# tsurumeso/vocal-remover

Measured on NVIDIA H100. Metric: seconds-of-audio/sec separated (n_fft=2048, hop=1024), higher is better.
Workload: dtype bf16x3 (split-bf16 operands hi+lo, 3 wgmma passes, fp32 accumulate); fft/lstm fp32

## Files before the change

vocal-remover_b200/build.py:

```python
import os
import subprocess
import sys
from concurrent.futures import ThreadPoolExecutor

HERE = os.path.dirname(os.path.abspath(__file__))
CSRC = os.path.join(HERE, 'csrc')
OBJ = os.path.join(HERE, 'build')
LIB = os.path.join(HERE, 'libvr_b200.so')
SOURCES = ['api.cu', 'engine.cu', 'conv_simt.cu', 'conv_tc.cu', 'conv_tc_rows.cu', 'conv_tc_halo.cu', 'elementwise.cu', 'lstm.cu', 'fft.cu', 'resample.cu']
NVCC = os.environ.get('NVCC', '/usr/local/cuda/bin/nvcc')
FLAGS = ['-gencode', 'arch=compute_90a,code=sm_90a', '-O3', '-lineinfo', '-std=c++17',
         '-Xcompiler', '-fPIC', '-Xcompiler', '-fvisibility=hidden', '--expt-relaxed-constexpr']


def _newest_header():
    hs = [os.path.join(CSRC, f) for f in os.listdir(CSRC) if f.endswith(('.h', '.cuh'))]
    hs.append(os.path.join(HERE, '..', 'include', 'vr_b200.h'))
    return max(os.path.getmtime(h) for h in hs)


def build(verbose=False, force=False):
    global OBJ, LIB
    extra = os.environ.get('VR_BUILD_FLAGS', '').split()
    if os.environ.get('VR_BUILD_TAG'):
        OBJ = os.path.join(HERE, 'build_' + os.environ['VR_BUILD_TAG'])
        LIB = os.path.join(HERE, 'libvr_b200_%s.so' % os.environ['VR_BUILD_TAG'])
    os.makedirs(OBJ, exist_ok=True)
    hdr = _newest_header()
    jobs = []
    for src in SOURCES:
        s = os.path.join(CSRC, src)
        o = os.path.join(OBJ, src.replace('.cu', '.o'))
        if force or not os.path.exists(o) or os.path.getmtime(o) < max(os.path.getmtime(s), hdr):
            jobs.append((s, o))

    def cc(job):
        s, o = job
        cmd = [NVCC] + FLAGS + extra + ['-c', s, '-o', o]
        if verbose:
            cmd += ['-Xptxas', '-v']
        r = subprocess.run(cmd, capture_output=True, text=True)
        if r.returncode != 0:
            raise RuntimeError('nvcc failed for %s:\n%s\n%s' % (s, r.stdout, r.stderr))
        return r.stderr

    with ThreadPoolExecutor(max_workers=min(8, max(1, len(jobs)))) as ex:
        logs = list(ex.map(cc, jobs))
    if verbose:
        for lg in logs:
            print(lg)
    objs = [os.path.join(OBJ, s.replace('.cu', '.o')) for s in SOURCES]
    if jobs or not os.path.exists(LIB):
        cmd = [NVCC, '-shared', '-o', LIB] + objs + ['-gencode', 'arch=compute_90a,code=sm_90a']
        r = subprocess.run(cmd, capture_output=True, text=True)
        if r.returncode != 0:
            raise RuntimeError('link failed:\n%s\n%s' % (r.stdout, r.stderr))
    return LIB


if __name__ == '__main__':
    print(build(verbose='-v' in sys.argv, force='-f' in sys.argv))
```

vocal-remover_b200/csrc/api.cu:

```cuda
#include <stdio.h>
#include <string.h>

#include <string>

#include "../../include/vr_b200.h"
#include "engine.h"
#include "kernels.h"
#include "tc_plan.h"

struct vr_ctx {
  vr::Engine* eng;
  std::string err;
};

static std::string g_create_err;

static int fail(vr_ctx* c, const std::string& m) {
  if (c) c->err = m;
  return -1;
}
static int done(vr_ctx* c, bool ok) {
  if (ok) return 0;
  c->err = c->eng->err;
  return -1;
}
#define CHECK_CTX(c) \
  if (!(c) || !(c)->eng) return -2;

extern "C" {

int vr_create(const vr_config* cfg, vr_ctx** out) {
  if (!cfg || !out) return -2;
  *out = nullptr;
  int ndev = 0;
  if (cudaGetDeviceCount(&ndev) != cudaSuccess || ndev == 0) {
    g_create_err = "no CUDA device visible: libvr_b200 has no CPU path";
    return -1;
  }
  if (cfg->device < 0 || cfg->device >= ndev) {
    g_create_err = "invalid device ordinal";
    return -1;
  }
  int nf = cfg->n_fft;
  if (nf < 64 || nf > 4096 || (nf & (nf - 1))) {
    g_create_err = "n_fft must be a power of two in [64, 4096]";
    return -1;
  }
  if (cfg->hop_length <= 0 || cfg->hop_length > nf) {
    g_create_err = "hop_length must be in (0, n_fft]";
    return -1;
  }
  if (cfg->max_batch <= 0 || cfg->cropsize <= 0) {
    g_create_err = "max_batch and cropsize must be positive";
    return -1;
  }
  vr::Config c;
  c.device = cfg->device; c.n_fft = cfg->n_fft; c.hop = cfg->hop_length; c.nout = cfg->nout;
  c.nout_lstm = cfg->nout_lstm; c.cropsize = cfg->cropsize; c.max_batch = cfg->max_batch;
  c.conv_mode = cfg->conv_mode;
  vr_ctx* ctx = new vr_ctx();
  ctx->eng = new vr::Engine(c);
  if (!ctx->eng->err.empty()) {
    g_create_err = ctx->eng->err;
    delete ctx->eng;
    delete ctx;
    return -1;
  }
  *out = ctx;
  return 0;
}

void vr_destroy(vr_ctx* ctx) {
  if (!ctx) return;
  delete ctx->eng;
  delete ctx;
}

const char* vr_last_error(const vr_ctx* ctx) { return ctx ? ctx->err.c_str() : g_create_err.c_str(); }

int vr_load_tensor(vr_ctx* ctx, const char* name, int32_t dtype, int32_t ndim, const int64_t* shape,
                   const void* host_data) {
  CHECK_CTX(ctx);
  if (!name || (!host_data) || ndim < 0 || ndim > 8) return fail(ctx, "vr_load_tensor: bad arguments");
  return done(ctx, ctx->eng->load_tensor(name, dtype, ndim, shape, host_data));
}

int vr_finalize_weights(vr_ctx* ctx) {
  CHECK_CTX(ctx);
  return done(ctx, ctx->eng->finalize());
}

int vr_stft(vr_ctx* ctx, const float* wave, int64_t L, void* spec, int64_t T, float* absmax, void* stream) {
  CHECK_CTX(ctx);
  return done(ctx, ctx->eng->stft(wave, L, (float2*)spec, T, absmax, (cudaStream_t)stream));
}

int vr_istft(vr_ctx* ctx, const void* spec, int64_t T, float* wave, void* stream) {
  CHECK_CTX(ctx);
  return done(ctx, ctx->eng->istft((const float2*)spec, nullptr, T, wave, nullptr, (cudaStream_t)stream));
}

int vr_predict_mask(vr_ctx* ctx, const float* mag, int32_t N, float* mask, void* stream) {
  CHECK_CTX(ctx);
  return done(ctx, ctx->eng->predict_mask(mag, N, mask, ctx->eng->cfg().offset, (cudaStream_t)stream));
}

int vr_forward(vr_ctx* ctx, const float* mag, int32_t N, float* mask, void* stream) {
  CHECK_CTX(ctx);
  return done(ctx, ctx->eng->predict_mask(mag, N, mask, 0, (cudaStream_t)stream));
}

int vr_normaliser(vr_ctx* ctx, const void* spec, int64_t T, int32_t norm_mode, float* out, void* stream) {
  CHECK_CTX(ctx);
  return done(ctx, ctx->eng->normaliser((const float2*)spec, T, norm_mode, out, (cudaStream_t)stream));
}

int vr_separate_windows(vr_ctx* ctx, const void* spec, int64_t T, const float* norm, int32_t pad_l,
                        int32_t first_window, int32_t n_windows, float* mask, int64_t mask_T, int64_t frame_shift,
                        int32_t accumulate, void* stream) {
  CHECK_CTX(ctx);
  return done(ctx, ctx->eng->separate_windows((const float2*)spec, T, norm, pad_l, first_window, n_windows, mask,
                                              mask_T, frame_shift, accumulate, (cudaStream_t)stream));
}

int vr_separate(vr_ctx* ctx, const void* spec, int64_t T, int32_t tta, float* mask, void* stream) {
  CHECK_CTX(ctx);
  return done(ctx, ctx->eng->separate((const float2*)spec, T, tta, mask, (cudaStream_t)stream));
}

int vr_apply_mask(vr_ctx* ctx, const void* spec, const float* mask, int64_t T, void* y_spec, void* v_spec,
                  void* stream) {
  CHECK_CTX(ctx);
  return done(ctx, ctx->eng->apply_mask((const float2*)spec, mask, T, (float2*)y_spec, (float2*)v_spec,
                                        (cudaStream_t)stream));
}

int vr_mask_frame_min(vr_ctx* ctx, const float* mask, int64_t T, float* frame_min, void* stream) {
  CHECK_CTX(ctx);
  return done(ctx, ctx->eng->mask_frame_min(mask, T, frame_min, (cudaStream_t)stream));
}

int vr_mask_apply_weight(vr_ctx* ctx, float* mask, int64_t T, const float* weight, void* stream) {
  CHECK_CTX(ctx);
  return done(ctx, ctx->eng->mask_apply_weight(mask, T, weight, (cudaStream_t)stream));
}

int vr_apply_mask_istft(vr_ctx* ctx, const void* spec, const float* mask, int64_t T, float* wave_inst,
                        float* wave_voc, void* stream) {
  CHECK_CTX(ctx);
  if (!mask) return fail(ctx, "vr_apply_mask_istft: mask is NULL");
  return done(ctx, ctx->eng->istft((const float2*)spec, mask, T, wave_inst, wave_voc, (cudaStream_t)stream));
}

int vr_stft_range(vr_ctx* ctx, const float* wave, int64_t L, void* spec, int64_t T, int64_t t0, int64_t t1,
                  void* stream) {
  CHECK_CTX(ctx);
  return done(ctx, ctx->eng->stft_range(wave, L, (float2*)spec, T, t0, t1, (cudaStream_t)stream));
}

int vr_normaliser_range(vr_ctx* ctx, const void* spec, int64_t T, int64_t t0, int64_t t1, float* out, void* stream) {
  CHECK_CTX(ctx);
  return done(ctx, ctx->eng->normaliser_range((const float2*)spec, T, t0, t1, out, (cudaStream_t)stream));
}

int vr_apply_mask_istft_range(vr_ctx* ctx, const void* spec, const float* mask, int64_t T, int64_t k0, int64_t k1,
                              float* wave_inst, float* wave_voc, void* stream) {
  CHECK_CTX(ctx);
  if (!mask) return fail(ctx, "vr_apply_mask_istft_range: mask is NULL");
  return done(ctx, ctx->eng->istft_range((const float2*)spec, mask, T, k0, k1, wave_inst, wave_voc,
                                         (cudaStream_t)stream));
}

int vr_separate_wave(vr_ctx* ctx, const float* wave, int64_t L, int32_t tta, float* wave_inst, float* wave_voc,
                     void* stream) {
  CHECK_CTX(ctx);
  return done(ctx, ctx->eng->separate_wave(wave, L, tta, wave_inst, wave_voc, (cudaStream_t)stream));
}

int vr_separate_wave_host(vr_ctx* ctx, const float* wave_host, int64_t L, int32_t tta, float* inst_host,
                          float* voc_host, void* stream) {
  CHECK_CTX(ctx);
  return done(ctx, ctx->eng->separate_wave_host(wave_host, L, tta, inst_host, voc_host, (cudaStream_t)stream));
}

int vr_separate_wave_host_images(vr_ctx* ctx, const float* wave_host, int64_t L, int32_t tta, float* inst_host,
                                 float* voc_host, uint8_t* img_inst_host, uint8_t* img_voc_host, void* stream) {
  CHECK_CTX(ctx);
  return done(ctx, ctx->eng->separate_wave_host(wave_host, L, tta, inst_host, voc_host, (cudaStream_t)stream,
                                                img_inst_host, img_voc_host));
}

int vr_spec_image(vr_ctx* ctx, const void* spec, const float* mask, int64_t T, uint8_t* img_a, uint8_t* img_b,
                  void* stream) {
  CHECK_CTX(ctx);
  return done(ctx, ctx->eng->spec_image((const float2*)spec, mask, T, img_a, img_b, (cudaStream_t)stream));
}

int vr_vocal_image(vr_ctx* ctx, const void* spec_x, const void* spec_y, int64_t T, uint8_t* img, void* stream) {
  CHECK_CTX(ctx);
  return done(ctx, ctx->eng->vocal_image((const float2*)spec_x, (const float2*)spec_y, T, img, (cudaStream_t)stream));
}

int vr_spec_sub(vr_ctx* ctx, const void* a, const void* b, int64_t T, void* out, void* stream) {
  CHECK_CTX(ctx);
  return done(ctx, ctx->eng->spec_sub((const float2*)a, (const float2*)b, T, (float2*)out, (cudaStream_t)stream));
}

int vr_validation_loss(vr_ctx* ctx, const void* spec_x, const void* spec_y, int64_t T, float* coef_out,
                       double* window_sums, void* stream) {
  CHECK_CTX(ctx);
  return done(ctx, ctx->eng->validation_loss((const float2*)spec_x, (const float2*)spec_y, T, coef_out, window_sums,
                                             (cudaStream_t)stream));
}

int vr_resample(vr_ctx* ctx, const float* x, int32_t channels, int64_t n_in, float* y, int64_t n_out, double sample_ratio,
                const double* win, const double* delta, int32_t nwin, int32_t table_per_crossing, void* stream) {
  auto bad = [&](const std::string& m) {
    if (ctx) return fail(ctx, m);
    g_create_err = m;
    return -1;
  };
  if (!x || !y || !win || !delta) return bad("vr_resample: null pointer");
  if (n_out != (int64_t)((double)n_in * sample_ratio))
    return bad("vr_resample: n_out must be int(n_in * sample_ratio) (resampy.core.resample)");
  if (ctx && ctx->eng) cudaSetDevice(ctx->eng->cfg().device);
  cudaError_t e = vr::launch_resample_sinc(x, channels, n_in, y, n_out, sample_ratio, win, delta, nwin, table_per_crossing,
                                           (cudaStream_t)stream);
  if (e != cudaSuccess) return bad(std::string("vr_resample: ") + cudaGetErrorString(e));
  return 0;
}

int vr_shared_alloc(vr_ctx* ctx, int64_t bytes, void** dev_ptr, unsigned char* handle64) {
  CHECK_CTX(ctx);
  if (!dev_ptr || !handle64 || bytes <= 0) return fail(ctx, "vr_shared_alloc: bad arguments");
  static_assert(sizeof(cudaIpcMemHandle_t) == 64, "CUDA IPC handle is 64 bytes");
  cudaSetDevice(ctx->eng->cfg().device);
  void* p = nullptr;
  cudaError_t e = cudaMalloc(&p, (size_t)bytes);
  if (e != cudaSuccess) return fail(ctx, std::string("vr_shared_alloc: cudaMalloc: ") + cudaGetErrorString(e));
  cudaIpcMemHandle_t h;
  e = cudaIpcGetMemHandle(&h, p);
  if (e != cudaSuccess) {
    cudaFree(p);
    return fail(ctx, std::string("vr_shared_alloc: cudaIpcGetMemHandle: ") + cudaGetErrorString(e));
  }
  memcpy(handle64, &h, 64);
  *dev_ptr = p;
  return 0;
}

int vr_shared_open(vr_ctx* ctx, const unsigned char* handle64, void** dev_ptr) {
  CHECK_CTX(ctx);
  if (!dev_ptr || !handle64) return fail(ctx, "vr_shared_open: bad arguments");
  cudaSetDevice(ctx->eng->cfg().device);
  cudaIpcMemHandle_t h;
  memcpy(&h, handle64, 64);
  void* p = nullptr;
  cudaError_t e = cudaIpcOpenMemHandle(&p, h, cudaIpcMemLazyEnablePeerAccess);
  if (e != cudaSuccess) return fail(ctx, std::string("vr_shared_open: cudaIpcOpenMemHandle: ") + cudaGetErrorString(e));
  *dev_ptr = p;
  return 0;
}

int vr_shared_close(vr_ctx* ctx, void* dev_ptr, int32_t owner) {
  CHECK_CTX(ctx);
  if (!dev_ptr) return 0;
  cudaSetDevice(ctx->eng->cfg().device);
  cudaError_t e = owner ? cudaFree(dev_ptr) : cudaIpcCloseMemHandle(dev_ptr);
  if (e != cudaSuccess) return fail(ctx, std::string("vr_shared_close: ") + cudaGetErrorString(e));
  return 0;
}

int64_t vr_launch_count(const vr_ctx* ctx) { return ctx && ctx->eng ? ctx->eng->launches : 0; }

int vr_profile_enable(vr_ctx* ctx, int32_t on) {
  CHECK_CTX(ctx);
  ctx->eng->profile_enable(on != 0);
  return 0;
}

int vr_profile_read(vr_ctx* ctx, double* out6) {
  CHECK_CTX(ctx);
  return done(ctx, ctx->eng->profile_read(out6));
}

int vr_profile_dump(vr_ctx* ctx, char* text, int64_t cap, int64_t* needed) {
  CHECK_CTX(ctx);
  std::string t;
  if (!ctx->eng->profile_dump(t)) return done(ctx, false);
  if (needed) *needed = (int64_t)t.size() + 1;
  if (text && cap > 0) {
    const size_t n = t.size() < (size_t)cap - 1 ? t.size() : (size_t)cap - 1;
    memcpy(text, t.data(), n);
    text[n] = 0;
  }
  return 0;
}

int vr_debug_conv(vr_ctx* ctx, const float* x, int32_t N, int32_t Cin, int32_t H, int32_t W, const float* w,
                  const float* bias, int32_t Cout, int32_t k, int32_t stride, int32_t dil_h, int32_t dil_w, int32_t act,
                  int32_t use_tc, float* y, void* stream) {
  CHECK_CTX(ctx);
  return done(ctx, ctx->eng->debug_conv(x, N, Cin, H, W, w, bias, Cout, k, stride, dil_h, dil_w, act, use_tc, y,
                                        (cudaStream_t)stream));
}

int vr_debug_decoder(vr_ctx* ctx, const float* low, int32_t N, int32_t Cl, int32_t h, int32_t w, const float* skip,
                     int32_t Cs, const float* wgt, const float* bias, int32_t Cout, int32_t act, int32_t fused, float* y,
                     void* stream) {
  CHECK_CTX(ctx);
  return done(ctx, ctx->eng->debug_decoder(low, N, Cl, h, w, skip, Cs, wgt, bias, Cout, act, fused, y,
                                           (cudaStream_t)stream));
}

int vr_debug_set(int32_t key, int32_t value) {
  int* knob = key == 0 ? &vr::g_debug.trace : key == 2 ? &vr::g_debug.rows_wide : key == 3 ? &vr::g_debug.halo
            : key == 6 ? &vr::g_debug.kskip : nullptr;
  if (!knob) return -1;
  *knob = value;
  return 0;
}

int64_t vr_debug_trace(uint64_t* host_out, int64_t capacity) {
  return vr::tc_rows_read_trace((unsigned long long*)host_out, (long long)capacity);
}

}
```

vocal-remover_b200/csrc/conv_tc.cu:

```cuda
#include <cuda.h>
#include <stdio.h>

#include <map>
#include <tuple>

#include "engine.h"
#include "tc_common.cuh"
#include "tc_plan.h"

namespace vr {

static constexpr int kMaxStages = 8;
static constexpr int kConsumerWarps = 8;
static constexpr int kThreads = 32 * kConsumerWarps + 32;

struct TcParams {
  int N, Ho, Wo, Wt, Ht, Nt, tiles_w, tiles_h, m_tiles, n_tiles;
  int stride, pad_h, pad_w, dil_h, dil_w, KW;
  int cchunks, total_sub, CinPadTC, Cout, act, stages;
  bf16* out_hi;
  bf16* out_lo;
  int64_t osn, osh;
  int osw;
  const float* bias;
};

template <int KB, int BN>
__global__ void __launch_bounds__(kThreads, 1)
    conv_tc_kernel(const __grid_constant__ CUtensorMap tmA, const __grid_constant__ CUtensorMap tmB, const TcParams p) {
  constexpr int SUBS = 64 / KB;
  constexpr int kSteps = KB / 16;
  constexpr uint32_t kAPlane = 128 * KB * 2;
  constexpr uint32_t kASub = 2 * kAPlane;
  constexpr uint32_t kBPlane = BN * KB * 2;
  constexpr uint32_t kBSub = 2 * kBPlane;
  constexpr uint32_t kStageBytes = SUBS * (kASub + kBSub);
  constexpr uint32_t kBRegion = SUBS * kASub;
  constexpr uint32_t kLayout = KB == 64 ? 1u : KB == 32 ? 2u : 3u;
  extern __shared__ uint8_t smem_raw[];
  __shared__ __align__(8) uint64_t bar_full[kMaxStages];
  __shared__ __align__(8) uint64_t bar_empty[kMaxStages];
  __shared__ float bias_s[256];

  const int warp = __shfl_sync(0xffffffffu, (int)threadIdx.x >> 5, 0);
  const int lane = threadIdx.x & 31;
  const uint32_t smem_base = (smem_u32(smem_raw) + 1023u) & ~1023u;
  const int total_tiles = p.m_tiles * p.n_tiles;
  const int num_iters = (p.total_sub + SUBS - 1) / SUBS;

  if (warp == kConsumerWarps && lane == 0) {
    asm volatile("prefetch.tensormap [%0];" ::"l"(&tmA) : "memory");
    asm volatile("prefetch.tensormap [%0];" ::"l"(&tmB) : "memory");
    for (int s = 0; s < p.stages; ++s) {
      mbar_init(smem_u32(&bar_full[s]), 1);
      mbar_init(smem_u32(&bar_empty[s]), kConsumerWarps);
    }
    asm volatile("fence.mbarrier_init.release.cluster;" ::: "memory");
  }
  for (int i = threadIdx.x; i < p.n_tiles * BN; i += blockDim.x) bias_s[i] = __ldg(p.bias + i);
  __syncthreads();

  if (warp == kConsumerWarps) {
    if (elect_one_sync()) {
      int stage = 0;
      uint32_t phase = 0;
      const uint32_t full0 = smem_u32(&bar_full[0]), empty0 = smem_u32(&bar_empty[0]);
      for (int tile = blockIdx.x; tile < total_tiles; tile += gridDim.x) {
        const int nt = tile % p.n_tiles;
        const int mt = tile / p.n_tiles;
        const int w0 = (mt % p.tiles_w) * p.Wt;
        const int h0 = ((mt / p.tiles_w) % p.tiles_h) * p.Ht;
        const int n0 = (mt / (p.tiles_w * p.tiles_h)) * p.Nt;
        const int wbase = w0 * p.stride - p.pad_w, hbase = h0 * p.stride - p.pad_h;
        const int nrow = nt * BN;
        int cc = 0, kw = 0, kh = 0, sub = 0;
        for (int it = 0; it < num_iters; ++it) {
          mbar_wait(empty0 + (uint32_t)stage * 8u, phase ^ 1u);
          const int nsub = min(SUBS, p.total_sub - sub);
          const uint32_t full = full0 + (uint32_t)stage * 8u;
          const uint32_t sbase = smem_base + (uint32_t)stage * kStageBytes;
          mbar_expect_tx(full, (uint32_t)nsub * (kASub + kBSub));
#pragma unroll
          for (int j = 0; j < SUBS; ++j) {
            if (j < nsub) {
              tma_load_5d(sbase + (uint32_t)j * kASub, &tmA, cc * KB, wbase + kw * p.dil_w, hbase + kh * p.dil_h, n0, 0, full);
              tma_load_3d(sbase + kBRegion + (uint32_t)j * kBSub, &tmB, (kh * p.KW + kw) * p.CinPadTC + cc * KB, nrow, 0,
                          full);
              ++sub;
              if (++cc == p.cchunks) {
                cc = 0;
                if (++kw == p.KW) {
                  kw = 0;
                  ++kh;
                }
              }
            }
          }
          if (++stage == p.stages) {
            stage = 0;
            phase ^= 1u;
          }
        }
      }
    }
    __syncwarp();
  } else {
    const int wg = warp >> 2;
    const float slope = p.act == ACT_RELU ? 0.f : p.act == ACT_LEAKY ? 0.01f : 1.f;
    const uint32_t dhi = desc_hi(8 * KB * 2, kLayout);
    const uint32_t full0 = smem_u32(&bar_full[0]), empty0 = smem_u32(&bar_empty[0]);
    int stage = 0;
    uint32_t phase = 0;
    float acc[BN / 2];
    for (int tile = blockIdx.x; tile < total_tiles; tile += gridDim.x) {
#pragma unroll
      for (int i = 0; i < BN / 2; ++i) acc[i] = 0.f;
      int prev = -1;
      for (int it = 0; it < num_iters; ++it) {
        const int nsub = min(SUBS, p.total_sub - it * SUBS);
        mbar_wait(full0 + (uint32_t)stage * 8u, phase);
        const uint32_t sdesc = desc_lo(smem_base + (uint32_t)stage * kStageBytes);
        wg_fence();
#pragma unroll
        for (int j = 0; j < SUBS; ++j) {
          if (j < nsub) {
            const uint32_t a_hi = sdesc + ((j * kASub + (uint32_t)wg * (kAPlane / 2)) >> 4);
            const uint32_t a_lo = a_hi + (kAPlane >> 4);
            const uint32_t b_hi = sdesc + ((kBRegion + j * kBSub) >> 4);
            const uint32_t b_lo = b_hi + (kBPlane >> 4);
#pragma unroll
            for (int k = 0; k < kSteps; ++k)
              wgmma_split3<BN>(acc, a_hi + 2u * k, a_lo + 2u * k, b_hi + 2u * k, b_lo + 2u * k, dhi);
          }
        }
        wg_commit();
        wg_wait<1>();
        if (prev >= 0) {
          __syncwarp();
          if (lane == 0) mbar_arrive(empty0 + (uint32_t)prev * 8u);
        }
        prev = stage;
        if (++stage == p.stages) {
          stage = 0;
          phase ^= 1u;
        }
      }
      wg_wait<0>();
      __syncwarp();
      if (lane == 0) mbar_arrive(empty0 + (uint32_t)prev * 8u);

      const int nt = tile % p.n_tiles;
      const int mt = tile / p.n_tiles;
      const int w0 = (mt % p.tiles_w) * p.Wt;
      const int h0 = ((mt / p.tiles_w) % p.tiles_h) * p.Ht;
      const int n0 = (mt / (p.tiles_w * p.tiles_h)) * p.Nt;
      const int c_lane = nt * BN + 2 * (lane & 3);
#pragma unroll
      for (int hr = 0; hr < 2; ++hr) {
        const int row = 64 * wg + 16 * (warp & 3) + (lane >> 2) + 8 * hr;
        const int dw = row % p.Wt;
        const int dh = (row / p.Wt) % p.Ht;
        const int n = n0 + row / (p.Wt * p.Ht);
        if (n >= p.N) continue;
        const int64_t obase = (int64_t)n * p.osn + (int64_t)(h0 + dh) * p.osh + (int64_t)(w0 + dw) * p.osw;
#pragma unroll
        for (int j = 0; j < BN / 8; ++j)
          epilogue_pair(acc[4 * j + 2 * hr], acc[4 * j + 2 * hr + 1], bias_s, c_lane + 8 * j, p.Cout, slope,
                        p.out_hi + obase, p.out_lo + obase);
      }
    }
  }
}

#define VR_TC_FOR_BN(X, KB) X(KB, 16) X(KB, 32) X(KB, 48) X(KB, 64) X(KB, 80) X(KB, 96) X(KB, 112) X(KB, 128)
#define VR_TC_FOR_ALL(X) VR_TC_FOR_BN(X, 64) VR_TC_FOR_BN(X, 32) VR_TC_FOR_BN(X, 16)


TcDebug g_debug;

static constexpr int kMaxDevices = 64;
const TcDevice& tc_device() {
  static TcDevice table[kMaxDevices];
  static TcDevice none;
  int dev = -1;
  if (cudaGetDevice(&dev) != cudaSuccess || dev < 0 || dev >= kMaxDevices) return none;
  TcDevice& d = table[dev];
  if (!d.ok) {
    if (cudaDeviceGetAttribute(&d.max_smem, cudaDevAttrMaxSharedMemoryPerBlockOptin, dev) != cudaSuccess ||
        cudaDeviceGetAttribute(&d.num_sms, cudaDevAttrMultiProcessorCount, dev) != cudaSuccess)
      return none;
#define VR_TC_SET_SMEM(KB, BN) \
  cudaFuncSetAttribute(conv_tc_kernel<KB, BN>, cudaFuncAttributeMaxDynamicSharedMemorySize, d.max_smem - 2048);
    VR_TC_FOR_ALL(VR_TC_SET_SMEM)
#undef VR_TC_SET_SMEM
    tc_rows_set_attributes(d.max_smem);
    tc_halo_set_attributes(d.max_smem);
    d.ok = true;
  }
  return d;
}

typedef CUresult (*EncodeTiledFn)(CUtensorMap*, CUtensorMapDataType, cuuint32_t, void*, const cuuint64_t*,
                                  const cuuint64_t*, const cuuint32_t*, const cuuint32_t*, CUtensorMapInterleave,
                                  CUtensorMapSwizzle, CUtensorMapL2promotion, CUtensorMapFloatOOBfill);
static EncodeTiledFn tc_encode_fn() {
  static EncodeTiledFn fn = nullptr;
  if (!fn) {
    void* p = nullptr;
    cudaDriverEntryPointQueryResult q;
    if (cudaGetDriverEntryPoint("cuTensorMapEncodeTiled", &p, cudaEnableDefault, &q) == cudaSuccess &&
        q == cudaDriverEntryPointSuccess)
      fn = (EncodeTiledFn)p;
  }
  return fn;
}

static CUtensorMapSwizzle swizzle_for(int KB) {
  return KB == 64 ? CU_TENSOR_MAP_SWIZZLE_128B : KB == 32 ? CU_TENSOR_MAP_SWIZZLE_64B : CU_TENSOR_MAP_SWIZZLE_32B;
}

static uint16_t tc_f2bf(float f) {
  uint32_t u;
  memcpy(&u, &f, 4);
  if ((u & 0x7fffffffu) > 0x7f800000u) return (uint16_t)((u >> 16) | 0x40);
  uint32_t r = 0x7fffu + ((u >> 16) & 1u);
  return (uint16_t)((u + r) >> 16);
}
static float tc_bf2f(uint16_t h) {
  uint32_t u = (uint32_t)h << 16;
  float f;
  memcpy(&f, &u, 4);
  return f;
}

struct TileGeom {
  int Wt, Ht, Nt;
  bool ok;
};
static TileGeom tile_geom(int Ho, int Wo) {
  TileGeom g{0, 0, 0, false};
  if (Wo <= 0 || Ho <= 0) return g;
  if (Wo >= 128) {
    if (Wo % 128) return g;
    g.Wt = 128; g.Ht = 1; g.Nt = 1;
  } else {
    if (128 % Wo) return g;
    g.Wt = Wo;
    g.Ht = 128 / Wo < Ho ? 128 / Wo : Ho;
    if (Ho % g.Ht) return g;
    if ((128 / Wo) % g.Ht) return g;
    g.Nt = 128 / (g.Wt * g.Ht);
  }
  g.ok = true;
  return g;
}

struct NTiling {
  int BN, n_tiles;
};
static NTiling n_tiling(const ConvLayer& L, bool rows) {
  const int cout16 = round_up(L.Cout, 16);
  if (rows) {
    const int BN = cout16 == 16 ? 16 : (L.rows_wide && cout16 % 64 == 0 ? 64 : 32);
    return {BN, ceil_div(cout16, BN)};
  }
  const int n_tiles = ceil_div(cout16, 128);
  return {round_up(ceil_div(cout16, n_tiles), 16), n_tiles};
}

static bool halo_has_bn(int BN) { return BN == 16 || BN == 32 || BN == 48 || BN == 64 || BN == 96 || BN == 128; }

TcKind tc_choose(const ConvLayer& L, int H, int W) {
  if (!(L.k == 1 || L.k == 3) || !(L.stride == 1 || L.stride == 2) || L.Cout < 4) return TC_NONE;
  const TileGeom g = tile_geom(H, W);
  if (!g.ok || g.Wt * L.stride > 256 || g.Ht * L.stride > 256) return TC_NONE;
  const bool k3s1 = L.k == 3 && L.stride == 1 && L.dil_h == 1 && L.dil_w == 1;
  const NTiling r = n_tiling(L, true), t = n_tiling(L, false);
  if (k3s1 && W % 128 == 0 && H % 8 == 0 && r.n_tiles * r.BN <= 256) return TC_ROWS;
  if (k3s1 && (W == 16 || W == 32 || W == 64) && H % (128 / W) == 0 && halo_has_bn(t.BN) &&
      t.n_tiles * t.BN <= 256 && g_debug.halo != 1)
    return TC_HALO;
  return TC_GENERIC;
}

template <class At>
static std::vector<uint16_t> split_bf16(const ConvLayer& L, int rows, int K, At at) {
  std::vector<uint16_t> planes((size_t)2 * rows * K, 0);
  const size_t lo = (size_t)rows * K;
  for (int co = 0; co < L.Cout; ++co)
    for (int t = 0; t < L.k * L.k; ++t)
      for (int ci = 0; ci < L.CinPad; ++ci) {
        const float w = L.w_host[((size_t)t * L.CinPad + ci) * L.CoutPad + co];
        const uint16_t hi = tc_f2bf(w);
        const size_t i = at(co, t, ci);
        planes[i] = hi;
        planes[lo + i] = tc_f2bf(w - tc_bf2f(hi));
      }
  return planes;
}

static unsigned long long weight_group_mask(const ConvLayer& L, int CinPad) {
  if (CinPad / 8 > 64) return ~0ull;
  unsigned long long m = 0x3ull;
  for (int ci = 0; ci < L.CinPad; ++ci) {
    bool any = false;
    for (int t = 0; t < L.k * L.k && !any; ++t)
      for (int co = 0; co < L.Cout && !any; ++co) any = L.w_host[((size_t)t * L.CinPad + ci) * L.CoutPad + co] != 0.f;
    if (any) m |= 1ull << (ci / 8);
  }
  return m;
}

static bool encode_weight_map(TcConv& tc, int rows, int K, int box_rows, std::string& err, const std::string& name) {
  cuuint64_t dims[3] = {(cuuint64_t)K, (cuuint64_t)rows, 2};
  cuuint64_t strides[2] = {(cuuint64_t)K * 2, (cuuint64_t)rows * K * 2};
  cuuint32_t box[3] = {(cuuint32_t)tc.KB, (cuuint32_t)box_rows, 2};
  cuuint32_t es[3] = {1, 1, 1};
  CUresult r = tc_encode_fn()(&tc.map_b, CU_TENSOR_MAP_DATA_TYPE_BFLOAT16, 3, tc.w_planes.get(), dims, strides, box, es,
                              CU_TENSOR_MAP_INTERLEAVE_NONE, swizzle_for(tc.KB), CU_TENSOR_MAP_L2_PROMOTION_L2_256B,
                              CU_TENSOR_MAP_FLOAT_OOB_FILL_NONE);
  if (r != CUDA_SUCCESS) {
    err = "cuTensorMapEncodeTiled(weights) failed for " + name + " code " + std::to_string((int)r);
    return false;
  }
  return true;
}

const CUtensorMap* tc_activation_map(TcConv& tc, const ActView& v, int bw, int bh, int bn, int es, std::string& err,
                                     const std::string& name) {
  const ViewKey key = std::make_tuple((const void*)v.hi, (const void*)v.lo, v.N, v.H, v.W, v.C, bw, bh, bn);
  auto it = tc.map_a.find(key);
  if (it != tc.map_a.end()) return &it->second;
  const int64_t plane = (const char*)v.lo - (const char*)v.hi;
  if (v.sw % 8 || v.sh % 8 || v.sn % 8 || (reinterpret_cast<uintptr_t>(v.hi) & 15) || plane <= 0 || plane % 16) {
    err = "internal: the input of " + name + " is not 16-byte aligned or its lo plane does not follow its hi plane";
    return nullptr;
  }
  cuuint64_t dims[5] = {(cuuint64_t)v.C, (cuuint64_t)v.W, (cuuint64_t)v.H, (cuuint64_t)v.N, 2};
  cuuint64_t strides[4] = {(cuuint64_t)v.sw * 2, (cuuint64_t)v.sh * 2, (cuuint64_t)v.sn * 2, (cuuint64_t)plane};
  cuuint32_t box[5] = {(cuuint32_t)tc.KB, (cuuint32_t)bw, (cuuint32_t)bh, (cuuint32_t)bn, 2};
  cuuint32_t estr[5] = {1, (cuuint32_t)es, (cuuint32_t)es, 1, 1};
  CUtensorMap m;
  CUresult r = tc_encode_fn()(&m, CU_TENSOR_MAP_DATA_TYPE_BFLOAT16, 5, (void*)v.hi, dims, strides, box, estr,
                              CU_TENSOR_MAP_INTERLEAVE_NONE, swizzle_for(tc.KB), CU_TENSOR_MAP_L2_PROMOTION_L2_256B,
                              CU_TENSOR_MAP_FLOAT_OOB_FILL_NONE);
  if (r != CUDA_SUCCESS) {
    err = "cuTensorMapEncodeTiled(activations) failed for " + name + " code " + std::to_string((int)r);
    return nullptr;
  }
  return &tc.map_a.emplace(key, m).first->second;
}

bool tc_prepare(ConvLayer& L, int H, int W, std::string& err) {
  const TcKind kind = tc_choose(L, H, W);
  if (kind == TC_NONE) return true;
  if (!tc_encode_fn()) {
    err = "cuTensorMapEncodeTiled is not available from the driver";
    return false;
  }
  auto tc = std::make_shared<TcConv>();
  tc->kind = kind;
  tc->H = H; tc->W = W;
  const NTiling nt = n_tiling(L, kind == TC_ROWS);
  const int BN = nt.BN, cin16 = round_up(L.CinPad, 16);
  tc->BN = BN; tc->n_tiles = nt.n_tiles;
  tc->KB = kind != TC_GENERIC ? 32 : cin16 % 64 == 0 ? 64 : cin16 % 32 == 0 ? 32 : 16;
  const int CinPad = round_up(L.CinPad, tc->KB);
  tc->CinPad = CinPad;
  tc->chunks = CinPad / tc->KB;
  tc->kmask = weight_group_mask(L, CinPad);
  const int rows = nt.n_tiles * BN;
  std::vector<uint16_t> planes;
  int brows, K;
  if (kind == TC_ROWS) {
    brows = 3 * rows;
    K = 3 * CinPad;
    planes = split_bf16(L, brows, K, [&](int co, int t, int ci) {
      return (size_t)(co / BN * 3 * BN + (2 - t / 3) * BN + co % BN) * K + (size_t)(t % 3) * CinPad + ci;
    });
  } else {
    brows = rows;
    K = L.k * L.k * CinPad;
    planes = split_bf16(L, brows, K, [&](int co, int t, int ci) { return (size_t)co * K + (size_t)t * CinPad + ci; });
  }
  std::vector<float> bias((size_t)rows, 0.f);
  for (int co = 0; co < L.Cout; ++co) bias[(size_t)co] = L.bias_host[(size_t)co];
  if (tc->w_planes.alloc(planes.size() * 2) != cudaSuccess || tc->bias.alloc(bias.size() * 4) != cudaSuccess) {
    err = "cudaMalloc failed while packing tensor-core weights for " + L.name;
    return false;
  }
  if (!upload(tc->w_planes.get(), planes.data(), planes.size() * 2, err) ||
      !upload(tc->bias.get(), bias.data(), bias.size() * 4, err) ||
      !encode_weight_map(*tc, brows, K, kind == TC_ROWS ? 3 * BN : BN, err, L.name))
    return false;
  L.tc = tc;
  return true;
}

cudaError_t tc_launch(ConvLayer& L, const ActView& in, const ActView& out, cudaStream_t s, std::string& err,
                      const ActView* up_src, const ActView* extra) {
  TcConv& tc = *L.tc;
  if (out.H != tc.H || out.W != tc.W || (in.H - 1) / L.stride + 1 != out.H || (in.W - 1) / L.stride + 1 != out.W) {
    err = "internal: " + L.name + " is launched on maps of another size than it was prepared for";
    return cudaErrorInvalidValue;
  }
  if (tc.kind == TC_ROWS) return tc_rows_launch(L, tc, in, out, s, err, up_src, extra);
  if (up_src || extra) {
    err = "tc_launch: fused upsample is only implemented in the row-streaming kernel";
    return cudaErrorInvalidValue;
  }
  if (tc.kind == TC_HALO) return tc_halo_launch(L, tc, in, out, s, err);
  const TileGeom g = tile_geom(out.H, out.W);
  const CUtensorMap* map_a = tc_activation_map(tc, in, g.Wt * L.stride, g.Ht * L.stride, g.Nt, L.stride, err, L.name);
  if (!map_a) return cudaErrorInvalidValue;
  const int SUBS = 64 / tc.KB;
  TcParams p;
  p.N = out.N; p.Ho = out.H; p.Wo = out.W;
  p.Wt = g.Wt; p.Ht = g.Ht; p.Nt = g.Nt;
  p.tiles_w = out.W / g.Wt; p.tiles_h = out.H / g.Ht;
  p.m_tiles = p.tiles_w * p.tiles_h * ceil_div(out.N, g.Nt);
  p.n_tiles = tc.n_tiles;
  p.stride = L.stride; p.dil_h = L.dil_h; p.dil_w = L.dil_w;
  p.pad_h = L.dil_h * (L.k / 2); p.pad_w = L.dil_w * (L.k / 2);
  p.KW = L.k;
  p.cchunks = tc.chunks; p.total_sub = L.k * L.k * tc.chunks;
  p.CinPadTC = tc.CinPad; p.Cout = L.Cout; p.act = L.act;
  const int stage_bytes = SUBS * (2 * 128 * tc.KB * 2 + 2 * tc.BN * tc.KB * 2);
  const TcDevice& dv = tc_device();
  if (!dv.ok) {
    err = "tc_launch: cannot query the current device";
    return cudaErrorInvalidValue;
  }
  const int dyn = dv.max_smem - 2048;
  p.stages = (dyn - 1024) / stage_bytes;
  if (p.stages > kMaxStages) p.stages = kMaxStages;
  if (p.stages < 2) {
    err = "tc_launch: shared memory too small for two pipeline stages";
    return cudaErrorInvalidValue;
  }
  p.out_hi = out.hi; p.out_lo = out.lo;
  p.osn = out.sn; p.osh = out.sh; p.osw = out.sw;
  p.bias = tc.bias.get();
  const int total_tiles = p.m_tiles * p.n_tiles;
  const int grid = total_tiles < dv.num_sms ? total_tiles : dv.num_sms;
#define VR_TC_LAUNCH(KB_, BN_)                                                       \
  if (tc.KB == KB_ && tc.BN == BN_) {                                                \
    conv_tc_kernel<KB_, BN_><<<grid, kThreads, dyn, s>>>(*map_a, tc.map_b, p);       \
    return cudaGetLastError();                                                       \
  }
  VR_TC_FOR_ALL(VR_TC_LAUNCH)
#undef VR_TC_LAUNCH
  err = "tc_launch: no kernel instantiation for this channel tile";
  return cudaErrorInvalidValue;
}

}
```

vocal-remover_b200/csrc/tc_plan.h:

```cpp
#pragma once
#include <cuda.h>

#include <map>
#include <tuple>

#include "engine.h"

namespace vr {

enum TcKind {
  TC_NONE,
  TC_GENERIC,
  TC_ROWS,
  TC_HALO,
};

typedef std::tuple<const void*, const void*, int, int, int, int, int, int, int> ViewKey;

struct TcConv {
  TcKind kind = TC_NONE;
  int H = 0, W = 0;
  int KB = 0, CinPad = 0, chunks = 0, BN = 0, n_tiles = 0;
  unsigned long long kmask = ~0ull;
  DevPtr<bf16> w_planes;
  DevPtr<float> bias;
  CUtensorMap map_b;
  std::map<ViewKey, CUtensorMap> map_a;
  bool fuses_upsample(int up_C) const { return kind == TC_ROWS && up_C % 32 == 0 && up_C <= CinPad; }
};

TcKind tc_choose(const ConvLayer& L, int H, int W);
const CUtensorMap* tc_activation_map(TcConv& tc, const ActView& v, int bw, int bh, int bn, int es, std::string& err,
                                     const std::string& name);

cudaError_t tc_rows_launch(ConvLayer& L, TcConv& tc, const ActView& in, const ActView& out, cudaStream_t s,
                           std::string& err, const ActView* up_src, const ActView* extra);
void tc_rows_set_attributes(int max_smem);
int tc_rows_read_trace(unsigned long long* out, long long capacity);

cudaError_t tc_halo_launch(ConvLayer& L, TcConv& tc, const ActView& in, const ActView& out, cudaStream_t s,
                           std::string& err);
void tc_halo_set_attributes(int max_smem);

struct TcDevice {
  bool ok = false;
  int num_sms = 0, max_smem = 0;
};
const TcDevice& tc_device();

struct TcDebug {
  int trace = 0;
  int rows_wide = 0;
  int halo = 0;
  int kskip = 1;
};
extern TcDebug g_debug;

}
```

Measured before the change: 2065.

## Add parity-split halo kernel for stride-2 3x3 tensor-core convolutions

Adds a dedicated warp-specialized wgmma kernel for 3x3 stride-2 convolutions. It loads the input tile once per channel chunk as four parity sub-grids via strided TMA and reuses them across all nine taps, instead of the generic per-tap im2col loads. Weights stay resident in shared memory when they fit. The cost is a new code path with its own smem budgeting and barriers, plus more complex selection logic.

```diff
diff --git a/vocal-remover_b200/build.py b/vocal-remover_b200/build.py
--- a/vocal-remover_b200/build.py
+++ b/vocal-remover_b200/build.py
@@ -7,7 +7,7 @@
 CSRC = os.path.join(HERE, 'csrc')
 OBJ = os.path.join(HERE, 'build')
 LIB = os.path.join(HERE, 'libvr_b200.so')
-SOURCES = ['api.cu', 'engine.cu', 'conv_simt.cu', 'conv_tc.cu', 'conv_tc_rows.cu', 'conv_tc_halo.cu', 'elementwise.cu', 'lstm.cu', 'fft.cu', 'resample.cu']
+SOURCES = ['api.cu', 'engine.cu', 'conv_simt.cu', 'conv_tc.cu', 'conv_tc_rows.cu', 'conv_tc_halo.cu', 'conv_tc_s2.cu', 'elementwise.cu', 'lstm.cu', 'fft.cu', 'resample.cu']
 NVCC = os.environ.get('NVCC', '/usr/local/cuda/bin/nvcc')
 FLAGS = ['-gencode', 'arch=compute_90a,code=sm_90a', '-O3', '-lineinfo', '-std=c++17',
          '-Xcompiler', '-fPIC', '-Xcompiler', '-fvisibility=hidden', '--expt-relaxed-constexpr']
diff --git a/vocal-remover_b200/csrc/api.cu b/vocal-remover_b200/csrc/api.cu
--- a/vocal-remover_b200/csrc/api.cu
+++ b/vocal-remover_b200/csrc/api.cu
@@ -315,7 +315,7 @@
 
 int vr_debug_set(int32_t key, int32_t value) {
   int* knob = key == 0 ? &vr::g_debug.trace : key == 2 ? &vr::g_debug.rows_wide : key == 3 ? &vr::g_debug.halo
-            : key == 6 ? &vr::g_debug.kskip : nullptr;
+            : key == 6 ? &vr::g_debug.kskip : key == 7 ? &vr::g_debug.s2 : nullptr;
   if (!knob) return -1;
   *knob = value;
   return 0;
diff --git a/vocal-remover_b200/csrc/conv_tc.cu b/vocal-remover_b200/csrc/conv_tc.cu
--- a/vocal-remover_b200/csrc/conv_tc.cu
+++ b/vocal-remover_b200/csrc/conv_tc.cu
@@ -195,6 +195,7 @@
 #undef VR_TC_SET_SMEM
     tc_rows_set_attributes(d.max_smem);
     tc_halo_set_attributes(d.max_smem);
+    tc_s2_set_attributes(d.max_smem);
     d.ok = true;
   }
   return d;
@@ -280,6 +281,9 @@
   if (k3s1 && (W == 16 || W == 32 || W == 64) && H % (128 / W) == 0 && halo_has_bn(t.BN) &&
       t.n_tiles * t.BN <= 256 && g_debug.halo != 1)
     return TC_HALO;
+  const bool k3s2 = L.k == 3 && L.stride == 2 && L.dil_h == 1 && L.dil_w == 1;
+  if (k3s2 && W % 16 == 0 && H % 8 == 0 && t.BN <= 64 && g_debug.s2 != 1)
+    return TC_S2;
   return TC_GENERIC;
 }
 
@@ -410,6 +414,7 @@
     return cudaErrorInvalidValue;
   }
   if (tc.kind == TC_HALO) return tc_halo_launch(L, tc, in, out, s, err);
+  if (tc.kind == TC_S2) return tc_s2_launch(L, tc, in, out, s, err);
   const TileGeom g = tile_geom(out.H, out.W);
   const CUtensorMap* map_a = tc_activation_map(tc, in, g.Wt * L.stride, g.Ht * L.stride, g.Nt, L.stride, err, L.name);
   if (!map_a) return cudaErrorInvalidValue;
diff --git a/vocal-remover_b200/csrc/conv_tc_s2.cu b/vocal-remover_b200/csrc/conv_tc_s2.cu
--- /dev/null
+++ b/vocal-remover_b200/csrc/conv_tc_s2.cu
@@ -0,0 +1,280 @@
+#include <stdio.h>
+
+#include "engine.h"
+#include "tc_common.cuh"
+#include "tc_plan.h"
+
+namespace vr {
+
+static constexpr int kConsumerWarps = 8;
+static constexpr int kThreads = 32 * (kConsumerWarps + 1);
+static constexpr int kHSlots = 2;
+static constexpr int kMaxWStages = 18;
+static constexpr uint32_t kKB = 32;
+static constexpr uint32_t kRowB = kKB * 2;
+static constexpr int kWt = 16, kHt = 8;
+
+struct S2Params {
+  int tiles_w, tiles_h, n_tiles, total_tiles;
+  int chunks, CinPadH, Cout, act, n_wstages;
+  int w_resident;
+  uint32_t hslot, htx;
+  uint32_t poff[4];
+  uint32_t plo[4];
+  uint32_t pw[4];
+  unsigned long long kmask;
+  bf16* out_hi;
+  bf16* out_lo;
+  int64_t osn, osh;
+  int osw;
+  const float* bias;
+};
+
+__device__ __forceinline__ uint32_t swz64(uint32_t q, uint32_t c) { return (q << 6) + ((c ^ ((q >> 1) & 3u)) << 4); }
+
+struct S2Tile {
+  int nt, h0, w0, n;
+};
+__device__ __forceinline__ S2Tile s2_tile(const S2Params& p, int tile) {
+  S2Tile t;
+  t.nt = tile % p.n_tiles;
+  const int mt = tile / p.n_tiles;
+  t.w0 = (mt % p.tiles_w) * kWt;
+  t.h0 = ((mt / p.tiles_w) % p.tiles_h) * kHt;
+  t.n = mt / (p.tiles_w * p.tiles_h);
+  return t;
+}
+
+template <int BN>
+__device__ __forceinline__ void consume_s2(int& hs, int& ws, int& pend_w, uint32_t& hph, uint32_t& wph,
+                                           const S2Params& p, float* acc, uint32_t (&fr)[2][8], const uint32_t* qb,
+                                           uint32_t h_base, uint32_t w_base, uint32_t dhi, uint32_t hfull0,
+                                           uint32_t hempty0, uint32_t wfull0, uint32_t wempty0, int lane) {
+  constexpr uint32_t kBPlane = BN * kRowB;
+  constexpr uint32_t kWStage = 2 * kBPlane;
+  mbar_wait(hfull0 + (uint32_t)hs * 8u, hph);
+  const uint32_t slot = h_base + (uint32_t)hs * p.hslot;
+#pragma unroll
+  for (int t = 0; t < 9; ++t) {
+    const int kh = t / 3, kw = t % 3;
+    const int P = 2 * (kh == 1) + (kw == 1);
+    const uint32_t q = qb[P] + (kh == 2 ? p.pw[P] : 0u) + (kw == 2 ? 1u : 0u);
+    const uint32_t box = slot + p.poff[P];
+#pragma unroll
+    for (int ks = 0; ks < 2; ++ks) {
+      uint32_t* f = fr[ks];
+      const uint32_t c = (uint32_t)(2 * ks) + ((uint32_t)lane >> 4);
+      ldsm_x4(f, box + swz64(q, c));
+      ldsm_x4(f + 4, box + swz64(q + p.plo[P], c));
+      if (ks == 0) mbar_wait(wfull0 + (uint32_t)ws * 8u, wph);
+      const uint32_t b_hi = desc_lo(w_base + (uint32_t)ws * kWStage) + (uint32_t)(ks * 32 >> 4);
+      wg_fence();
+      wgmma_split3_rs<BN>(acc, f, f + 4, b_hi, b_hi + (kBPlane >> 4), dhi);
+      wg_commit();
+      if (t == 8 && ks == 1) {
+        __syncwarp();
+        if (lane == 0) mbar_arrive(hempty0 + (uint32_t)hs * 8u);
+      }
+      wg_wait<1>();
+      if (pend_w >= 0) {
+        __syncwarp();
+        if (lane == 0) mbar_arrive(wempty0 + (uint32_t)pend_w * 8u);
+        pend_w = -1;
+      }
+    }
+    pend_w = ws;
+    if (++ws == p.n_wstages) {
+      ws = 0;
+      if (!p.w_resident) wph ^= 1u;
+    }
+  }
+  if (++hs == kHSlots) {
+    hs = 0;
+    hph ^= 1u;
+  }
+}
+
+template <int BN>
+__global__ void __launch_bounds__(kThreads, 1)
+    conv_tc_s2_kernel(const __grid_constant__ CUtensorMap tmA0, const __grid_constant__ CUtensorMap tmA1,
+                      const __grid_constant__ CUtensorMap tmA2, const __grid_constant__ CUtensorMap tmA3,
+                      const __grid_constant__ CUtensorMap tmB, const S2Params p) {
+  constexpr uint32_t kWStage = 2 * BN * kRowB;
+  extern __shared__ uint8_t smem_raw[];
+  __shared__ __align__(8) uint64_t bar_hfull[kHSlots];
+  __shared__ __align__(8) uint64_t bar_hempty[kHSlots];
+  __shared__ __align__(8) uint64_t bar_wfull[kMaxWStages];
+  __shared__ __align__(8) uint64_t bar_wempty[kMaxWStages];
+  __shared__ float bias_s[256];
+
+  const int warp = __shfl_sync(0xffffffffu, (int)threadIdx.x >> 5, 0);
+  const int lane = threadIdx.x & 31;
+  const uint32_t smem_base = (smem_u32(smem_raw) + 1023u) & ~1023u;
+  const uint32_t h_base = smem_base;
+  const uint32_t w_base = smem_base + (uint32_t)kHSlots * p.hslot;
+
+  if (warp == kConsumerWarps && lane == 0) {
+    asm volatile("prefetch.tensormap [%0];" ::"l"(&tmA0) : "memory");
+    asm volatile("prefetch.tensormap [%0];" ::"l"(&tmA1) : "memory");
+    asm volatile("prefetch.tensormap [%0];" ::"l"(&tmA2) : "memory");
+    asm volatile("prefetch.tensormap [%0];" ::"l"(&tmA3) : "memory");
+    asm volatile("prefetch.tensormap [%0];" ::"l"(&tmB) : "memory");
+    for (int s = 0; s < kHSlots; ++s) {
+      mbar_init(smem_u32(&bar_hfull[s]), 1);
+      mbar_init(smem_u32(&bar_hempty[s]), kConsumerWarps);
+    }
+    for (int s = 0; s < p.n_wstages; ++s) {
+      mbar_init(smem_u32(&bar_wfull[s]), 1);
+      mbar_init(smem_u32(&bar_wempty[s]), kConsumerWarps);
+    }
+    asm volatile("fence.mbarrier_init.release.cluster;" ::: "memory");
+  }
+  for (int i = threadIdx.x; i < p.n_tiles * BN; i += blockDim.x) bias_s[i] = __ldg(p.bias + i);
+  __syncthreads();
+  const uint32_t hfull0 = smem_u32(&bar_hfull[0]), hempty0 = smem_u32(&bar_hempty[0]);
+  const uint32_t wfull0 = smem_u32(&bar_wfull[0]), wempty0 = smem_u32(&bar_wempty[0]);
+
+  if (warp == kConsumerWarps) {
+    if (elect_one_sync()) {
+      int hs = 0, ws = 0;
+      uint32_t hph = 0, wph = 0;
+      for (int tile = blockIdx.x; tile < p.total_tiles; tile += gridDim.x) {
+        const S2Tile tl = s2_tile(p, tile);
+        for (int cc = 0; cc < p.chunks; ++cc) {
+          if (!chunk_groups(p.kmask, cc)) continue;
+          mbar_wait(hempty0 + (uint32_t)hs * 8u, hph ^ 1u);
+          const uint32_t hfull = hfull0 + (uint32_t)hs * 8u;
+          const uint32_t slot = h_base + (uint32_t)hs * p.hslot;
+          mbar_expect_tx(hfull, p.htx);
+          const int c0 = cc * (int)kKB, wo = 2 * tl.w0 - 1, ho = 2 * tl.h0 - 1;
+          tma_load_5d(slot + p.poff[0], &tmA0, c0, wo, ho, tl.n, 0, hfull);
+          tma_load_5d(slot + p.poff[1], &tmA1, c0, wo + 1, ho, tl.n, 0, hfull);
+          tma_load_5d(slot + p.poff[2], &tmA2, c0, wo, ho + 1, tl.n, 0, hfull);
+          tma_load_5d(slot + p.poff[3], &tmA3, c0, wo + 1, ho + 1, tl.n, 0, hfull);
+          if (++hs == kHSlots) {
+            hs = 0;
+            hph ^= 1u;
+          }
+          for (int t = 0; t < 9 && (!p.w_resident || tile == (int)blockIdx.x); ++t) {
+            mbar_wait(wempty0 + (uint32_t)ws * 8u, wph ^ 1u);
+            const uint32_t wfull = wfull0 + (uint32_t)ws * 8u;
+            mbar_expect_tx(wfull, kWStage);
+            tma_load_3d(w_base + (uint32_t)ws * kWStage, &tmB, t * p.CinPadH + cc * (int)kKB, tl.nt * BN, 0, wfull);
+            if (++ws == p.n_wstages) {
+              ws = 0;
+              wph ^= 1u;
+            }
+          }
+        }
+      }
+    }
+    __syncwarp();
+  } else {
+    const int wg = warp >> 2;
+    const float slope = p.act == ACT_RELU ? 0.f : p.act == ACT_LEAKY ? 0.01f : 1.f;
+    const uint32_t dhi = desc_hi(8 * kRowB, 2u);
+    const int px = 64 * wg + 16 * (warp & 3) + (lane & 15);
+    const uint32_t i = (uint32_t)(px / kWt), j = (uint32_t)(px % kWt);
+    uint32_t qb[4];
+#pragma unroll
+    for (int P = 0; P < 4; ++P) qb[P] = i * p.pw[P] + j;
+    int hs = 0, ws = 0, pend_w = -1;
+    uint32_t hph = 0, wph = 0;
+    float acc[BN / 2];
+    uint32_t fr[2][8];
+    for (int tile = blockIdx.x; tile < p.total_tiles; tile += gridDim.x) {
+#pragma unroll
+      for (int k = 0; k < BN / 2; ++k) acc[k] = 0.f;
+      for (int cc = 0; cc < p.chunks; ++cc) {
+        if (!chunk_groups(p.kmask, cc)) continue;
+        consume_s2<BN>(hs, ws, pend_w, hph, wph, p, acc, fr, qb, h_base, w_base, dhi, hfull0, hempty0, wfull0, wempty0,
+                       lane);
+      }
+      wg_wait<0>();
+      __syncwarp();
+      if (lane == 0 && pend_w >= 0) mbar_arrive(wempty0 + (uint32_t)pend_w * 8u);
+      pend_w = -1;
+
+      const S2Tile tl = s2_tile(p, tile);
+      const int c_lane = tl.nt * BN + 2 * (lane & 3);
+#pragma unroll
+      for (int hr = 0; hr < 2; ++hr) {
+        const int po = 64 * wg + 16 * (warp & 3) + (lane >> 2) + 8 * hr;
+        const int64_t obase = (int64_t)tl.n * p.osn + (int64_t)(tl.h0 + po / kWt) * p.osh +
+                              (int64_t)(tl.w0 + po % kWt) * p.osw;
+        const float* v = acc + 2 * hr;
+#pragma unroll
+        for (int jj = 0; jj < BN / 8; ++jj)
+          epilogue_pair(v[4 * jj], v[4 * jj + 1], bias_s, c_lane + 8 * jj, p.Cout, slope, p.out_hi + obase,
+                        p.out_lo + obase);
+      }
+    }
+  }
+}
+
+#define VR_S2_FOR_ALL(X) X(16) X(32) X(48) X(64)
+
+cudaError_t tc_s2_launch(ConvLayer& L, TcConv& tc, const ActView& in, const ActView& out, cudaStream_t s,
+                         std::string& err) {
+  const TcDevice& dv = tc_device();
+  if (!dv.ok) {
+    err = "tc_s2_launch: cannot query the current device";
+    return cudaErrorInvalidValue;
+  }
+  S2Params p;
+  p.tiles_w = out.W / kWt;
+  p.tiles_h = out.H / kHt;
+  p.n_tiles = tc.n_tiles;
+  p.total_tiles = out.N * p.tiles_h * p.tiles_w * p.n_tiles;
+  p.chunks = tc.chunks; p.CinPadH = tc.CinPad; p.Cout = L.Cout; p.act = L.act;
+  p.kmask = g_debug.kskip == 1 ? tc.kmask : ~0ull;
+  p.out_hi = out.hi; p.out_lo = out.lo;
+  p.osn = out.sn; p.osh = out.sh; p.osw = out.sw;
+  p.bias = tc.bias.get();
+  const CUtensorMap* maps[4];
+  p.hslot = 0;
+  p.htx = 0;
+  for (int P = 0; P < 4; ++P) {
+    const int bh = kHt + 1 - (P >> 1), bw = kWt + 1 - (P & 1);
+    maps[P] = tc_activation_map(tc, in, 2 * bw, 2 * bh, 1, 2, err, L.name);
+    if (!maps[P]) return cudaErrorInvalidValue;
+    p.pw[P] = (uint32_t)bw;
+    p.plo[P] = (uint32_t)(bh * bw);
+    p.poff[P] = p.hslot;
+    const uint32_t bytes = 2u * p.plo[P] * kRowB;
+    p.htx += bytes;
+    p.hslot += (uint32_t)round_up((int)bytes, 512);
+  }
+  const int w_stage = tc.BN * 2 * (int)kRowB;
+  const int dyn = dv.max_smem - 2048;
+  const int avail = dyn - 1024;
+  p.n_wstages = (avail - kHSlots * (int)p.hslot) / w_stage;
+  int live_chunks = 0;
+  for (int cc = 0; cc < tc.chunks; ++cc) live_chunks += (cc * 4 + 4 <= 64 ? (p.kmask >> (cc * 4)) & 0xFu : 0xFu) != 0;
+  p.w_resident = 9 * live_chunks <= kMaxWStages && 9 * live_chunks <= p.n_wstages;
+  if (p.w_resident) p.n_wstages = 9 * live_chunks;
+  if (p.n_wstages > kMaxWStages) p.n_wstages = kMaxWStages;
+  if (p.n_wstages < 2) {
+    err = "tc_s2_launch: shared memory too small for two parity slots and two weight stages";
+    return cudaErrorInvalidValue;
+  }
+  const int grid = p.total_tiles < dv.num_sms ? p.total_tiles : dv.num_sms;
+#define VR_S2_LAUNCH(BN_)                                                                                   \
+  if (tc.BN == BN_) {                                                                                       \
+    conv_tc_s2_kernel<BN_><<<grid, kThreads, dyn, s>>>(*maps[0], *maps[1], *maps[2], *maps[3], tc.map_b, p); \
+    return cudaGetLastError();                                                                              \
+  }
+  VR_S2_FOR_ALL(VR_S2_LAUNCH)
+#undef VR_S2_LAUNCH
+  err = "tc_s2_launch: no kernel instantiation for this channel tile";
+  return cudaErrorInvalidValue;
+}
+
+void tc_s2_set_attributes(int max_smem) {
+#define VR_S2_SET(BN_) \
+  cudaFuncSetAttribute(conv_tc_s2_kernel<BN_>, cudaFuncAttributeMaxDynamicSharedMemorySize, max_smem - 2048);
+  VR_S2_FOR_ALL(VR_S2_SET)
+#undef VR_S2_SET
+}
+
+}
diff --git a/vocal-remover_b200/csrc/tc_plan.h b/vocal-remover_b200/csrc/tc_plan.h
--- a/vocal-remover_b200/csrc/tc_plan.h
+++ b/vocal-remover_b200/csrc/tc_plan.h
@@ -13,6 +13,7 @@
   TC_GENERIC,
   TC_ROWS,
   TC_HALO,
+  TC_S2,
 };
 
 typedef std::tuple<const void*, const void*, int, int, int, int, int, int, int> ViewKey;
@@ -42,6 +43,10 @@
                            std::string& err);
 void tc_halo_set_attributes(int max_smem);
 
+cudaError_t tc_s2_launch(ConvLayer& L, TcConv& tc, const ActView& in, const ActView& out, cudaStream_t s,
+                         std::string& err);
+void tc_s2_set_attributes(int max_smem);
+
 struct TcDevice {
   bool ok = false;
   int num_sms = 0, max_smem = 0;
@@ -53,6 +58,7 @@
   int rows_wide = 0;
   int halo = 0;
   int kskip = 1;
+  int s2 = 0;
 };
 extern TcDebug g_debug;
 
```

New measurement: 2098 (median of 6 runs). 1.02x the previous value.
